# Alandroid/img-compression-mps

Hardware: AMD Instinct MI355X
Metric: Mvoxels/s compress+reconstruct, 256^3 fp32, bond chi=64; SSIM vs ref (higher is better)
Workload: dtype f32

## Files before the change

img-compression-mps_amd/csrc/gemm.hip:

```cpp
#include <stdlib.h>

#include <algorithm>

#include <mutex>
#include <type_traits>

#include "common.h"

namespace {

typedef float f32x16 __attribute__((ext_vector_type(16)));
typedef double f64x4 __attribute__((ext_vector_type(4)));

template <typename T>
struct Mfma;

template <>
struct Mfma<float> {
  static constexpr int MT = 32;
  static constexpr int KS = 2;
  static constexpr int NACC = 16;
  typedef f32x16 acc_t;
  static __device__ __forceinline__ acc_t mma(float a, float b, acc_t c) {
    return __builtin_amdgcn_mfma_f32_32x32x2f32(a, b, c, 0, 0, 0);
  }
  static __device__ __forceinline__ int acc_row(int reg, int lane) {
    return (reg & 3) + 8 * (reg >> 2) + 4 * (lane >> 5);
  }
  static __device__ __forceinline__ int acc_col(int lane) { return lane & 31; }
  static __device__ __forceinline__ int frag_idx(int lane) { return lane & 31; }
  static __device__ __forceinline__ int frag_k(int lane) { return lane >> 5; }
};

template <>
struct Mfma<double> {
  static constexpr int MT = 16;
  static constexpr int KS = 4;
  static constexpr int NACC = 4;
  typedef f64x4 acc_t;
  static __device__ __forceinline__ acc_t mma(double a, double b, acc_t c) {
    return __builtin_amdgcn_mfma_f64_16x16x4f64(a, b, c, 0, 0, 0);
  }
  static __device__ __forceinline__ int acc_row(int reg, int lane) { return (lane >> 4) + 4 * reg; }
  static __device__ __forceinline__ int acc_col(int lane) { return lane & 15; }
  static __device__ __forceinline__ int frag_idx(int lane) { return lane & 15; }
  static __device__ __forceinline__ int frag_k(int lane) { return lane >> 4; }
};

template <typename T>
struct alignas(sizeof(T) * 4) Quad {
  T v[4];
};

struct GemmIndex {
  const int64_t* a_row;
  const int64_t* a_col;
  const int64_t* c_row;
  const int64_t* c_col;
  int guarded;
};
inline int gemm_guarded_env() { return getenv("NDMPS_GEMM_GUARDED") ? 1 : 0; }

constexpr int kGemmMaxBatch = 64;
struct GemmBatchPtrs {
  const void* a[kGemmMaxBatch];
  const void* b[kGemmMaxBatch];
  void* c[kGemmMaxBatch];
};

template <typename T, int BM, int BN, int WAVES_M, int WAVES_N, bool TA, bool TB, bool VEC, bool IDX>
__device__ __forceinline__ void
gemm_body(int64_t M, int64_t N, int64_t K, const T* __restrict__ A, int64_t lda, const T* __restrict__ B, int64_t ldb,
          T* __restrict__ C, int64_t ldc, const GemmIndex& ix) {
  using MF = Mfma<T>;
  constexpr int BK = 16;
  constexpr int MT = MF::MT;
  constexpr int TM = BM / (WAVES_M * MT);
  constexpr int TN = BN / (WAVES_N * MT);
  constexpr int PAD = 4;
  constexpr int A_PER = BM * BK / 256, B_PER = BN * BK / 256;
  static_assert(WAVES_M * WAVES_N == 4, "4 waves per workgroup");
  static_assert(TM >= 1 && TN >= 1, "tile too small");
  constexpr bool VA = VEC && A_PER % 4 == 0, VB = VEC && B_PER % 4 == 0;

  __shared__ T As[BK][BM + PAD];
  __shared__ T Bs[BK][BN + PAD];

  const int tid = threadIdx.x;
  const int lane = tid & 63;
  const int wave = tid >> 6;
  const int wm = wave / WAVES_N;
  const int wn = wave % WAVES_N;
  const int64_t m0 = (int64_t)blockIdx.x * BM;
  const int64_t n0 = (int64_t)blockIdx.y * BN;

  typename MF::acc_t acc[TM][TN];
#pragma unroll
  for (int i = 0; i < TM; ++i)
#pragma unroll
    for (int j = 0; j < TN; ++j)
#pragma unroll
      for (int r = 0; r < MF::NACC; ++r) acc[i][j][r] = (T)0;

  T ra[A_PER], rb[B_PER];

  constexpr int kIdxK = 1024;
  __shared__ int64_t acol_s[(IDX && !TA && VEC) ? kIdxK : 1];
  int64_t arow_q[(A_PER / 4) > 0 ? (A_PER / 4) : 1];
  const bool idx_fast = IDX && !TA && VA && ix.a_row != nullptr && K <= kIdxK;
  if (IDX && !TA && VA) {
    if (idx_fast) {
      for (int64_t kk = tid; kk < K; kk += 256) acol_s[kk] = ix.a_col[kk];
#pragma unroll
      for (int i = 0; i < A_PER / 4; ++i) {
        const int m = (tid + 256 * i) / (BK / 4);
        arow_q[i] = m0 + m < M ? ix.a_row[m0 + m] : 0;
      }
      __syncthreads();
    }
  }

  const bool inner_a = VA && m0 + BM <= M && !ix.guarded, inner_b = VB && n0 + BN <= N && !ix.guarded;
  auto fetch_a = [&](int64_t k0) {
    if (VA && inner_a && k0 + BK <= K) {
#pragma unroll
      for (int i = 0; i < A_PER / 4; ++i) {
        const int e = tid + 256 * i;
        const T* src;
        if (TA) {
          src = A + (k0 + e / (BM / 4)) * lda + m0 + (e % (BM / 4)) * 4;
        } else {
          const int m = e / (BK / 4), k = (e % (BK / 4)) * 4;
          if (IDX && idx_fast) src = A + arow_q[i] + acol_s[k0 + k];
          else if (IDX && ix.a_row) src = A + ix.a_row[m0 + m] + ix.a_col[k0 + k];
          else src = A + (m0 + m) * lda + k0 + k;
        }
        const Quad<T> q = *reinterpret_cast<const Quad<T>*>(src);
#pragma unroll
        for (int j = 0; j < 4; ++j) ra[4 * i + j] = q.v[j];
      }
    } else if (VA) {
#pragma unroll
      for (int i = 0; i < A_PER / 4; ++i) {
        const int e = tid + 256 * i;
        Quad<T> q;
        q.v[0] = q.v[1] = q.v[2] = q.v[3] = (T)0;
        if (TA) {
          const int k = e / (BM / 4), m = (e % (BM / 4)) * 4;
          if (k0 + k < K && m0 + m < M) q = *reinterpret_cast<const Quad<T>*>(A + (k0 + k) * lda + m0 + m);
        } else {
          const int m = e / (BK / 4), k = (e % (BK / 4)) * 4;
          if (k0 + k < K && m0 + m < M) {
            if (IDX && idx_fast) q = *reinterpret_cast<const Quad<T>*>(A + arow_q[i] + acol_s[k0 + k]);
            else if (IDX && ix.a_row) q = *reinterpret_cast<const Quad<T>*>(A + ix.a_row[m0 + m] + ix.a_col[k0 + k]);
            else q = *reinterpret_cast<const Quad<T>*>(A + (m0 + m) * lda + k0 + k);
          }
        }
#pragma unroll
        for (int j = 0; j < 4; ++j) ra[4 * i + j] = q.v[j];
      }
    } else {
#pragma unroll
      for (int i = 0; i < A_PER; ++i) {
        const int e = tid + 256 * i;
        int m, k;
        if (TA) {
          k = e / BM;
          m = e % BM;
        } else {
          m = e / BK;
          k = e % BK;
        }
        const int64_t gk = k0 + k, gm = m0 + m;
        if (IDX && ix.a_row) ra[i] = (gk < K && gm < M) ? A[ix.a_row[gm] + ix.a_col[gk]] : (T)0;
        else ra[i] = (gk < K && gm < M) ? (TA ? A[gk * lda + gm] : A[gm * lda + gk]) : (T)0;
      }
    }
  };
  auto fetch_b = [&](int64_t k0) {
    if (VB && inner_b && k0 + BK <= K) {
#pragma unroll
      for (int i = 0; i < B_PER / 4; ++i) {
        const int e = tid + 256 * i;
        const T* src = TB ? B + (n0 + e / (BK / 4)) * ldb + k0 + (e % (BK / 4)) * 4
                          : B + (k0 + e / (BN / 4)) * ldb + n0 + (e % (BN / 4)) * 4;
        const Quad<T> q = *reinterpret_cast<const Quad<T>*>(src);
#pragma unroll
        for (int j = 0; j < 4; ++j) rb[4 * i + j] = q.v[j];
      }
    } else if (VB) {
#pragma unroll
      for (int i = 0; i < B_PER / 4; ++i) {
        const int e = tid + 256 * i;
        Quad<T> q;
        q.v[0] = q.v[1] = q.v[2] = q.v[3] = (T)0;
        if (TB) {
          const int n = e / (BK / 4), k = (e % (BK / 4)) * 4;
          if (k0 + k < K && n0 + n < N) q = *reinterpret_cast<const Quad<T>*>(B + (n0 + n) * ldb + k0 + k);
        } else {
          const int k = e / (BN / 4), n = (e % (BN / 4)) * 4;
          if (k0 + k < K && n0 + n < N) q = *reinterpret_cast<const Quad<T>*>(B + (k0 + k) * ldb + n0 + n);
        }
#pragma unroll
        for (int j = 0; j < 4; ++j) rb[4 * i + j] = q.v[j];
      }
    } else {
#pragma unroll
      for (int i = 0; i < B_PER; ++i) {
        const int e = tid + 256 * i;
        int n, k;
        if (TB) {
          n = e / BK;
          k = e % BK;
        } else {
          k = e / BN;
          n = e % BN;
        }
        const int64_t gk = k0 + k, gn = n0 + n;
        rb[i] = (gk < K && gn < N) ? (TB ? B[gn * ldb + gk] : B[gk * ldb + gn]) : (T)0;
      }
    }
  };
  auto commit = [&]() {
    if (VA) {
#pragma unroll
      for (int i = 0; i < A_PER / 4; ++i) {
        const int e = tid + 256 * i;
        if (TA) {
          const int k = e / (BM / 4), m = (e % (BM / 4)) * 4;
#pragma unroll
          for (int j = 0; j < 4; ++j) As[k][m + j] = ra[4 * i + j];
        } else {
          const int m = e / (BK / 4), k = (e % (BK / 4)) * 4;
#pragma unroll
          for (int j = 0; j < 4; ++j) As[k + j][m] = ra[4 * i + j];
        }
      }
    } else {
#pragma unroll
      for (int i = 0; i < A_PER; ++i) {
        const int e = tid + 256 * i;
        if (TA) As[e / BM][e % BM] = ra[i];
        else As[e % BK][e / BK] = ra[i];
      }
    }
    if (VB) {
#pragma unroll
      for (int i = 0; i < B_PER / 4; ++i) {
        const int e = tid + 256 * i;
        if (TB) {
          const int n = e / (BK / 4), k = (e % (BK / 4)) * 4;
#pragma unroll
          for (int j = 0; j < 4; ++j) Bs[k + j][n] = rb[4 * i + j];
        } else {
          const int k = e / (BN / 4), n = (e % (BN / 4)) * 4;
#pragma unroll
          for (int j = 0; j < 4; ++j) Bs[k][n + j] = rb[4 * i + j];
        }
      }
    } else {
#pragma unroll
      for (int i = 0; i < B_PER; ++i) {
        const int e = tid + 256 * i;
        if (TB) Bs[e % BK][e / BK] = rb[i];
        else Bs[e / BN][e % BN] = rb[i];
      }
    }
  };

  fetch_a(0);
  fetch_b(0);
  const int fi = MF::frag_idx(lane);
  const int fk = MF::frag_k(lane);
  for (int64_t k0 = 0; k0 < K; k0 += BK) {
    __syncthreads();
    commit();
    __syncthreads();
    if (k0 + BK < K) {
      fetch_a(k0 + BK);
      fetch_b(k0 + BK);
    }
#pragma unroll
    for (int kk = 0; kk < BK; kk += MF::KS) {
      T a[TM], b[TN];
#pragma unroll
      for (int i = 0; i < TM; ++i) a[i] = As[kk + fk][(wm * TM + i) * MT + fi];
#pragma unroll
      for (int j = 0; j < TN; ++j) b[j] = Bs[kk + fk][(wn * TN + j) * MT + fi];
#pragma unroll
      for (int i = 0; i < TM; ++i)
#pragma unroll
        for (int j = 0; j < TN; ++j) acc[i][j] = MF::mma(a[i], b[j], acc[i][j]);
    }
  }

  if constexpr (IDX && MF::MT == 32 && BM == 128 && BN == 128 && sizeof(T) == 4) {
    if (ix.c_row) {
      __shared__ float cstage[4][32][36];
      float (*st)[36] = cstage[wave];
      const int rl0 = lane >> 3, cl = (lane & 7) * 4;
      int64_t roff[TM][4], coff[TN][4];
#pragma unroll
      for (int j = 0; j < TN; ++j) {
        const int64_t col = n0 + (wn * TN + j) * MT + cl;
#pragma unroll
        for (int e = 0; e < 4; ++e) coff[j][e] = col + e < N ? ix.c_col[col + e] : -1;
      }
#pragma unroll
      for (int i = 0; i < TM; ++i)
#pragma unroll
        for (int ps = 0; ps < 4; ++ps) {
          const int64_t row = m0 + (wm * TM + i) * MT + rl0 + 8 * ps;
          roff[i][ps] = row < M ? ix.c_row[row] : -1;
        }
#pragma unroll
      for (int i = 0; i < TM; ++i)
#pragma unroll
        for (int j = 0; j < TN; ++j) {
#pragma unroll
          for (int r = 0; r < MF::NACC; ++r) st[MF::acc_row(r, lane)][MF::acc_col(lane)] = acc[i][j][r];
          __builtin_amdgcn_fence(__ATOMIC_RELEASE, "wavefront");
          __builtin_amdgcn_wave_barrier();
          __builtin_amdgcn_fence(__ATOMIC_ACQUIRE, "wavefront");
          const bool run = coff[j][0] >= 0 && coff[j][3] == coff[j][0] + 3 && coff[j][1] == coff[j][0] + 1 &&
                           coff[j][2] == coff[j][0] + 2;
#pragma unroll
          for (int ps = 0; ps < 4; ++ps) {
            const float4 v = *reinterpret_cast<const float4*>(&st[rl0 + 8 * ps][cl]);
            const int64_t ro = roff[i][ps];
            if (ro < 0) continue;
            if (run && ((ro + coff[j][0]) & 3) == 0) {
              *reinterpret_cast<float4*>(C + ro + coff[j][0]) = v;
            } else {
              if (coff[j][0] >= 0) C[ro + coff[j][0]] = v.x;
              if (coff[j][1] >= 0) C[ro + coff[j][1]] = v.y;
              if (coff[j][2] >= 0) C[ro + coff[j][2]] = v.z;
              if (coff[j][3] >= 0) C[ro + coff[j][3]] = v.w;
            }
          }
          __builtin_amdgcn_fence(__ATOMIC_RELEASE, "wavefront");
          __builtin_amdgcn_wave_barrier();
        }
      return;
    }
  }
  if (IDX && ix.c_row) {
    int64_t roff[TM][MF::NACC], coff[TN];
#pragma unroll
    for (int j = 0; j < TN; ++j) {
      const int64_t col = n0 + (wn * TN + j) * MT + MF::acc_col(lane);
      coff[j] = col < N ? ix.c_col[col] : -1;
    }
#pragma unroll
    for (int i = 0; i < TM; ++i)
#pragma unroll
      for (int r = 0; r < MF::NACC; ++r) {
        const int64_t row = m0 + (wm * TM + i) * MT + MF::acc_row(r, lane);
        roff[i][r] = row < M ? ix.c_row[row] : -1;
      }
#pragma unroll
    for (int i = 0; i < TM; ++i)
#pragma unroll
      for (int j = 0; j < TN; ++j)
#pragma unroll
        for (int r = 0; r < MF::NACC; ++r)
          if (roff[i][r] >= 0 && coff[j] >= 0) C[roff[i][r] + coff[j]] = acc[i][j][r];
    return;
  }
#pragma unroll
  for (int i = 0; i < TM; ++i)
#pragma unroll
    for (int j = 0; j < TN; ++j) {
      const int64_t col = n0 + (wn * TN + j) * MT + MF::acc_col(lane);
#pragma unroll
      for (int r = 0; r < MF::NACC; ++r) {
        const int64_t row = m0 + (wm * TM + i) * MT + MF::acc_row(r, lane);
        if (row < M && col < N) C[row * ldc + col] = acc[i][j][r];
      }
    }
}

template <typename T, int BM, int BN, int WAVES_M, int WAVES_N, bool TA, bool TB, bool VEC, bool IDX = false>
__global__ void __launch_bounds__(256, 2)
gemm_kernel(int64_t M, int64_t N, int64_t K, const T* __restrict__ A, int64_t lda,
            const T* __restrict__ B, int64_t ldb, T* __restrict__ C, int64_t ldc, GemmIndex ix = GemmIndex()) {
  gemm_body<T, BM, BN, WAVES_M, WAVES_N, TA, TB, VEC, IDX>(M, N, K, A, lda, B, ldb, C, ldc, ix);
}

template <typename T, int BM, int BN, int WAVES_M, int WAVES_N, bool TA, bool TB, bool VEC, bool IDX = false>
__global__ void __launch_bounds__(256, 2)
gemm_batched_kernel(int64_t M, int64_t N, int64_t K, GemmBatchPtrs p, int64_t lda, int64_t ldb, int64_t ldc,
                    GemmIndex ix = GemmIndex()) {
  gemm_body<T, BM, BN, WAVES_M, WAVES_N, TA, TB, VEC, IDX>(M, N, K, static_cast<const T*>(p.a[blockIdx.z]), lda,
                                                           static_cast<const T*>(p.b[blockIdx.z]), ldb,
                                                           static_cast<T*>(p.c[blockIdx.z]), ldc, ix);
}

template <typename T, int BM, int BN, int WAVES_M, int WAVES_N>
int launch_gemm(int transA, int transB, int64_t m, int64_t n, int64_t k, const T* A, int64_t lda,
                const T* B, int64_t ldb, T* C, int64_t ldc, hipStream_t stream, const GemmBatchPtrs* bp = nullptr,
                int batch = 1) {
  dim3 grid((unsigned)ndmps::ceil_div(m, BM), (unsigned)ndmps::ceil_div(n, BN), (unsigned)batch);
  dim3 block(256);
  GemmIndex gi{nullptr, nullptr, nullptr, nullptr, gemm_guarded_env()};
  const uintptr_t al = sizeof(T) * 4;
  bool vec = lda % 4 == 0 && ldb % 4 == 0 && k % 4 == 0 && (!transA || m % 4 == 0) && (transB || n % 4 == 0);
  if (bp) {
    for (int z = 0; z < batch; ++z) vec = vec && (uintptr_t)bp->a[z] % al == 0 && (uintptr_t)bp->b[z] % al == 0;
  } else {
    vec = vec && (uintptr_t)A % al == 0 && (uintptr_t)B % al == 0;
  }
#define NDMPS_GEMM_LAUNCH(TA_, TB_, V_)                                                                            \
  do {                                                                                                              \
    if (bp)                                                                                                         \
      hipLaunchKernelGGL((gemm_batched_kernel<T, BM, BN, WAVES_M, WAVES_N, TA_, TB_, V_>), grid, block, 0, stream,  \
                         m, n, k, *bp, lda, ldb, ldc, gi);                                                          \
    else                                                                                                            \
      hipLaunchKernelGGL((gemm_kernel<T, BM, BN, WAVES_M, WAVES_N, TA_, TB_, V_>), grid, block, 0, stream, m, n, k,  \
                         A, lda, B, ldb, C, ldc, gi);                                                               \
  } while (0)
#define NDMPS_GEMM_TRANS(V_)                                     \
  do {                                                           \
    if (transA && transB) NDMPS_GEMM_LAUNCH(true, true, V_);     \
    else if (transA) NDMPS_GEMM_LAUNCH(true, false, V_);         \
    else if (transB) NDMPS_GEMM_LAUNCH(false, true, V_);         \
    else NDMPS_GEMM_LAUNCH(false, false, V_);                    \
  } while (0)
  if (vec) NDMPS_GEMM_TRANS(true);
  else NDMPS_GEMM_TRANS(false);
#undef NDMPS_GEMM_TRANS
#undef NDMPS_GEMM_LAUNCH
  NDMPS_LAUNCH_CHECK();
  return NDMPS_OK;
}

template <typename T>
int gemm_check(int64_t m, int64_t n, int64_t k, const T* A, int64_t lda, int transA, const T* B,
               int64_t ldb, int transB, T* C, int64_t ldc) {
  NDMPS_REQUIRE(m >= 0 && n >= 0 && k >= 0, "negative GEMM extent");
  NDMPS_REQUIRE(A && B && C, "NULL GEMM operand");
  NDMPS_REQUIRE(lda >= (transA ? m : k) && ldb >= (transB ? k : n) && ldc >= n,
                "leading dimension too small (lda=%lld ldb=%lld ldc=%lld)", (long long)lda,
                (long long)ldb, (long long)ldc);
  NDMPS_REQUIRE(ndmps::ceil_div(n, 16) < 65536, "GEMM n=%lld exceeds grid.y", (long long)n);
  NDMPS_REQUIRE(ndmps::ceil_div(m, 32) < 2147483647LL, "GEMM m=%lld exceeds grid.x", (long long)m);
  return NDMPS_OK;
}

template <int T, typename TIN>
__global__ void __launch_bounds__(256, 2)
gram_partial_kernel(const TIN* __restrict__ A, int64_t m, int64_t n, int64_t lda,
                    double* __restrict__ partial, int n_tiles_1d, int64_t rows_per_slab) {
  constexpr int TS = 16 * T;
  __shared__ double red[TS][TS + 1];

  int tile = blockIdx.x, ti = 0;
  while (tile >= n_tiles_1d - ti) {
    tile -= n_tiles_1d - ti;
    ++ti;
  }
  const int tj = ti + tile;
  const int64_t i0 = (int64_t)ti * TS, j0 = (int64_t)tj * TS;
  const int64_t slab = blockIdx.y;
  const int64_t r_begin = slab * rows_per_slab;
  const int64_t r_end = min(m, r_begin + rows_per_slab);

  const int tid = threadIdx.x, lane = tid & 63, wave = tid >> 6;
  const int lr = lane >> 4, lc = lane & 15;

  f64x4 acc[T][T];
#pragma unroll
  for (int a = 0; a < T; ++a)
#pragma unroll
    for (int b = 0; b < T; ++b) acc[a][b] = (f64x4){0.0, 0.0, 0.0, 0.0};

  for (int64_t r = r_begin + 4 * wave; r < r_end; r += 16) {
    const int64_t row = r + lr;
    const bool row_ok = row < r_end;
    double av[T], bv[T];
#pragma unroll
    for (int a = 0; a < T; ++a) {
      const int64_t ca = i0 + 16 * a + lc;
      const int64_t cb = j0 + 16 * a + lc;
      av[a] = (row_ok && ca < n) ? ndmps::to_f64(A[row * lda + ca]) : 0.0;
      bv[a] = (row_ok && cb < n) ? ndmps::to_f64(A[row * lda + cb]) : 0.0;
    }
#pragma unroll
    for (int a = 0; a < T; ++a)
#pragma unroll
      for (int b = 0; b < T; ++b)
        acc[a][b] = __builtin_amdgcn_mfma_f64_16x16x4f64(av[a], bv[b], acc[a][b], 0, 0, 0);
  }

  for (int w = 0; w < 4; ++w) {
    if (wave == w) {
#pragma unroll
      for (int a = 0; a < T; ++a)
#pragma unroll
        for (int b = 0; b < T; ++b)
#pragma unroll
          for (int reg = 0; reg < 4; ++reg) {
            const int rr = 16 * a + lr + 4 * reg, cc = 16 * b + lc;
            if (w == 0) red[rr][cc] = acc[a][b][reg];
            else red[rr][cc] += acc[a][b][reg];
          }
    }
    __syncthreads();
  }
  double* out = partial + ((int64_t)slab * gridDim.x + blockIdx.x) * (TS * TS);
  for (int e = tid; e < TS * TS; e += 256) out[e] = red[e / TS][e % TS];
}

template <int TS>
__global__ void __launch_bounds__(256)
tile_reduce_kernel(const double* __restrict__ partial, int n_slabs, int per_group, int n_tiles_1d,
                   int n_tiles, double* __restrict__ out, double* __restrict__ G, int64_t n, int final,
                   const int32_t* __restrict__ perm = nullptr) {
  const int e = blockIdx.y * 256 + threadIdx.x;
  if (e >= TS * TS) return;
  const int s0 = blockIdx.z * per_group, s1 = min(n_slabs, s0 + per_group);
  const double* src = partial + (int64_t)blockIdx.x * (TS * TS) + e;
  const int64_t slab_stride = (int64_t)n_tiles * (TS * TS);
  double s = 0.0;
  int sl = s0;
  for (; sl + 4 <= s1; sl += 4) {
    const double v0 = src[(sl + 0) * slab_stride], v1 = src[(sl + 1) * slab_stride];
    const double v2 = src[(sl + 2) * slab_stride], v3 = src[(sl + 3) * slab_stride];
    s = (((s + v0) + v1) + v2) + v3;
  }
  for (; sl < s1; ++sl) s += src[sl * slab_stride];
  if (!final) {
    out[((int64_t)blockIdx.z * n_tiles + blockIdx.x) * (TS * TS) + e] = s;
    return;
  }
  int tile = blockIdx.x, ti = 0;
  while (tile >= n_tiles_1d - ti) {
    tile -= n_tiles_1d - ti;
    ++ti;
  }
  const int tj = ti + tile;
  const int64_t r = (int64_t)ti * TS + e / TS, c = (int64_t)tj * TS + e % TS;
  if (r < n && c < n && (ti != tj || c >= r)) {
    const int64_t pr = perm ? perm[r] : r, pc = perm ? perm[c] : c;
    G[pr * n + pc] = s;
    G[pc * n + pr] = s;
  }
// ... 525 lines not shown
    for (int a = 0; a < (ROLE == 2 ? 2 : 4); ++a)
#pragma unroll
      for (int b = 0; b < 4; ++b) {
        if (ROLE == 1 && a > b) continue;
#pragma unroll
        for (int reg = 0; reg < 4; ++reg) {
          const int rr = a_col + 16 * a + lr + 4 * reg, cc = b_col + 16 * b + lc;
          out[rr * 128 + cc] = acc[4 * a + b][reg];
        }
      }
  };
  if (!diag) run(std::integral_constant<int, 0>{});
  else if (wave == 0 || wave == 3) run(std::integral_constant<int, 1>{});
  else run(std::integral_constant<int, 2>{});
}

__global__ void __launch_bounds__(256)
gram128_reduce_kernel(const double* __restrict__ partial, Gram128Geom g, double* __restrict__ G, int64_t stride_G, int64_t n,
                      const int32_t* __restrict__ perm) {
  const int e = blockIdx.y * 256 + threadIdx.x;
  const int t = blockIdx.x;
  int ti, tj, base, count;
  if (t < g.n_off) {
    int u = t;
    ti = 0;
    while (u >= g.tiles_1d - 1 - ti) {
      u -= g.tiles_1d - 1 - ti;
      ++ti;
    }
    tj = ti + 1 + u;
    base = t * g.slabs_off;
    count = g.slabs_off;
  } else {
    ti = tj = t - g.n_off;
    base = g.n_off * g.slabs_off + (t - g.n_off) * g.slabs_diag;
    count = g.slabs_diag;
  }
  const int64_t r = (int64_t)ti * 128 + e / 128, c = (int64_t)tj * 128 + e % 128;
  if (r >= n || c >= n || (ti == tj && c < r)) return;
  const double* src = partial + ((int64_t)blockIdx.z * g.slots + base) * (128 * 128) + e;
  double s = 0.0;
  int sl = 0;
  for (; sl + 4 <= count; sl += 4) {
    const double v0 = src[(int64_t)(sl + 0) * 16384], v1 = src[(int64_t)(sl + 1) * 16384];
    const double v2 = src[(int64_t)(sl + 2) * 16384], v3 = src[(int64_t)(sl + 3) * 16384];
    s = (((s + v0) + v1) + v2) + v3;
  }
  for (; sl < count; ++sl) s += src[(int64_t)sl * 16384];
  double* Gb = G + (int64_t)blockIdx.z * stride_G;
  const int64_t pr = perm ? perm[r] : r, pc = perm ? perm[c] : c;
  Gb[pr * n + pc] = s;
  Gb[pc * n + pr] = s;
}

template <typename TIN>
__global__ void __launch_bounds__(256)
gram_small_kernel(const TIN* __restrict__ A, int64_t m, int n, int64_t lda, double* __restrict__ partial,
                  int vec_ok) {
  __shared__ double red[4][36];
  double acc[36];
#pragma unroll
  for (int i = 0; i < 36; ++i) acc[i] = 0.0;
  const int64_t stride = (int64_t)gridDim.x * 256;
  for (int64_t r = (int64_t)blockIdx.x * 256 + threadIdx.x; r < m; r += stride) {
    float x[8];
    const TIN* row = A + r * lda;
    if (vec_ok) {
      const float4 a = load4_as_f32(row), b = load4_as_f32(row + 4);
      x[0] = a.x; x[1] = a.y; x[2] = a.z; x[3] = a.w; x[4] = b.x; x[5] = b.y; x[6] = b.z; x[7] = b.w;
    } else {
#pragma unroll
      for (int c = 0; c < 8; ++c) x[c] = c < n ? (float)row[c] : 0.f;
    }
    int idx = 0;
#pragma unroll
    for (int i = 0; i < 8; ++i)
#pragma unroll
      for (int j = i; j < 8; ++j) acc[idx++] += (double)x[i] * (double)x[j];
  }
#pragma unroll
  for (int i = 0; i < 36; ++i) {
    double v = acc[i];
    for (int off = 32; off > 0; off >>= 1) v += __shfl_down(v, off, 64);
    if ((threadIdx.x & 63) == 0) red[threadIdx.x >> 6][i] = v;
  }
  __syncthreads();
  if (threadIdx.x < 36)
    partial[(int64_t)blockIdx.x * 36 + threadIdx.x] =
        (red[0][threadIdx.x] + red[1][threadIdx.x]) + (red[2][threadIdx.x] + red[3][threadIdx.x]);
}

__global__ void __launch_bounds__(256)
gram_small_reduce_kernel(const double* __restrict__ partial, int n_blocks, double* __restrict__ G, int n) {
  __shared__ double part[7][36];
  const int e = threadIdx.x % 36, grp = threadIdx.x / 36;
  if (grp < 7) {
    double acc = 0.0;
    for (int b = grp; b < n_blocks; b += 7) acc += partial[(int64_t)b * 36 + e];
    part[grp][e] = acc;
  }
  __syncthreads();
  if (threadIdx.x >= 36) return;
  double s = 0.0;
  for (int k = 0; k < 7; ++k) s += part[k][e];
  int i = 0, rem = e;
  while (rem >= 8 - i) {
    rem -= 8 - i;
    ++i;
  }
  const int j = i + rem;
  if (i < n && j < n) {
    G[i * n + j] = s;
    G[j * n + i] = s;
  }
}

constexpr int kGramSmallBlocks = 256;

struct GramGeom {
  int T;
  int tiles_1d;
  int n_tiles;
  int n_slabs;
  int64_t rows_per_slab;
};

GramGeom gram_geometry(int64_t m, int64_t n) {
  GramGeom g;
  g.T = n <= 16 ? 1 : (n <= 32 ? 2 : 4);
  const int ts = 16 * g.T;
  g.tiles_1d = (int)ndmps::ceil_div(n, ts);
  g.n_tiles = g.tiles_1d * (g.tiles_1d + 1) / 2;
  int64_t want = std::max<int64_t>(1, (2 * ndmps::kNumCU) / g.n_tiles);
  int64_t rows = ndmps::round_up(std::max<int64_t>(ndmps::ceil_div(m, want), 64), 16);
  g.rows_per_slab = rows;
  g.n_slabs = (int)std::max<int64_t>(1, ndmps::ceil_div(m, rows));
  return g;
}

}

extern "C" int ndmps_sgemm(int transA, int transB, int64_t m, int64_t n, int64_t k, const float* d_A,
                           int64_t lda, const float* d_B, int64_t ldb, float* d_C, int64_t ldc,
                           ndmps_stream_t stream) {
  NDMPS_TRY(gemm_check(m, n, k, d_A, lda, transA, d_B, ldb, transB, d_C, ldc));
  if (m == 0 || n == 0) return NDMPS_OK;
  hipStream_t s = (hipStream_t)stream;
  if (n <= 32) return launch_gemm<float, 128, 32, 4, 1>(transA, transB, m, n, k, d_A, lda, d_B, ldb, d_C, ldc, s);
  if (n <= 64 || m <= 64)
    return launch_gemm<float, 64, 64, 2, 2>(transA, transB, m, n, k, d_A, lda, d_B, ldb, d_C, ldc, s);
  return launch_gemm<float, 128, 128, 2, 2>(transA, transB, m, n, k, d_A, lda, d_B, ldb, d_C, ldc, s);
}

extern "C" int ndmps_sgemm_indexed(int64_t m, int64_t n, int64_t k, const float* d_A, int64_t lda,
                                   const int64_t* d_a_row, const int64_t* d_a_col, int a_vec4, const float* d_B,
                                   int64_t ldb, float* d_C, int64_t ldc, const int64_t* d_c_row,
                                   const int64_t* d_c_col, ndmps_stream_t stream) {
  NDMPS_REQUIRE(m >= 0 && n >= 0 && k >= 0 && d_A && d_B && d_C, "bad indexed GEMM argument");
  NDMPS_REQUIRE((d_a_row == nullptr) == (d_a_col == nullptr) && (d_c_row == nullptr) == (d_c_col == nullptr),
                "offset tables come in (row, column) pairs");
  NDMPS_REQUIRE(ldb >= n && (d_a_row || lda >= k) && (d_c_row || ldc >= n), "leading dimension too small");
  if (m == 0 || n == 0) return NDMPS_OK;
  hipStream_t s = (hipStream_t)stream;
  GemmIndex ix{d_a_row, d_a_col, d_c_row, d_c_col, gemm_guarded_env()};
  const uintptr_t al = 16;
  const bool vec = ldb % 4 == 0 && k % 4 == 0 && n % 4 == 0 && (uintptr_t)d_A % al == 0 && (uintptr_t)d_B % al == 0 &&
                   (d_a_row ? a_vec4 != 0 : lda % 4 == 0);
  const dim3 block(256);
  if (n <= 64 || m <= 64) {
    const dim3 grid((unsigned)ndmps::ceil_div(m, 64), (unsigned)ndmps::ceil_div(n, 64));
    if (vec)
      hipLaunchKernelGGL((gemm_kernel<float, 64, 64, 2, 2, false, false, true, true>), grid, block, 0, s, m, n, k, d_A,
                         lda, d_B, ldb, d_C, ldc, ix);
    else
      hipLaunchKernelGGL((gemm_kernel<float, 64, 64, 2, 2, false, false, false, true>), grid, block, 0, s, m, n, k, d_A,
                         lda, d_B, ldb, d_C, ldc, ix);
  } else {
    const dim3 grid((unsigned)ndmps::ceil_div(m, 128), (unsigned)ndmps::ceil_div(n, 128));
    if (vec)
      hipLaunchKernelGGL((gemm_kernel<float, 128, 128, 2, 2, false, false, true, true>), grid, block, 0, s, m, n, k,
                         d_A, lda, d_B, ldb, d_C, ldc, ix);
    else
      hipLaunchKernelGGL((gemm_kernel<float, 128, 128, 2, 2, false, false, false, true>), grid, block, 0, s, m, n, k,
                         d_A, lda, d_B, ldb, d_C, ldc, ix);
  }
  NDMPS_LAUNCH_CHECK();
  return NDMPS_OK;
}

extern "C" int ndmps_dgemm(int transA, int transB, int64_t m, int64_t n, int64_t k, const double* d_A,
                           int64_t lda, const double* d_B, int64_t ldb, double* d_C, int64_t ldc,
                           ndmps_stream_t stream) {
  NDMPS_TRY(gemm_check(m, n, k, d_A, lda, transA, d_B, ldb, transB, d_C, ldc));
  if (m == 0 || n == 0) return NDMPS_OK;
  hipStream_t s = (hipStream_t)stream;
  if (n <= 16) return launch_gemm<double, 64, 16, 4, 1>(transA, transB, m, n, k, d_A, lda, d_B, ldb, d_C, ldc, s);
  if (n <= 32 || m <= 32)
    return launch_gemm<double, 32, 32, 2, 2>(transA, transB, m, n, k, d_A, lda, d_B, ldb, d_C, ldc, s);
  return launch_gemm<double, 64, 64, 2, 2>(transA, transB, m, n, k, d_A, lda, d_B, ldb, d_C, ldc, s);
}

namespace {
template <typename T>
int gemm_batched_check(int batch, const T* const* h_A, const T* const* h_B, T* const* h_C, GemmBatchPtrs& bp) {
  NDMPS_REQUIRE(batch >= 1 && batch <= kGemmMaxBatch && h_A && h_B && h_C, "batched GEMM: batch=%d outside [1, %d] or NULL array",
                batch, kGemmMaxBatch);
  for (int z = 0; z < batch; ++z) {
    NDMPS_REQUIRE(h_A[z] && h_B[z] && h_C[z], "batched GEMM: NULL operand %d", z);
    bp.a[z] = h_A[z];
    bp.b[z] = h_B[z];
    bp.c[z] = h_C[z];
  }
  return NDMPS_OK;
}
}

extern "C" int ndmps_gemm_batched_max(void) { return kGemmMaxBatch; }

extern "C" int ndmps_sgemm_batched(int batch, int transA, int transB, int64_t m, int64_t n, int64_t k,
                                   const float* const* h_A, int64_t lda, const float* const* h_B, int64_t ldb,
                                   float* const* h_C, int64_t ldc, ndmps_stream_t stream) {
  GemmBatchPtrs bp;
  NDMPS_TRY(gemm_batched_check(batch, h_A, h_B, h_C, bp));
  NDMPS_TRY(gemm_check(m, n, k, h_A[0], lda, transA, h_B[0], ldb, transB, h_C[0], ldc));
  if (m == 0 || n == 0) return NDMPS_OK;
  hipStream_t s = (hipStream_t)stream;
  const float* A = nullptr;
  float* Cn = nullptr;
  if (n <= 32) return launch_gemm<float, 128, 32, 4, 1>(transA, transB, m, n, k, A, lda, A, ldb, Cn, ldc, s, &bp, batch);
  if (n <= 64 || m <= 64)
    return launch_gemm<float, 64, 64, 2, 2>(transA, transB, m, n, k, A, lda, A, ldb, Cn, ldc, s, &bp, batch);
  return launch_gemm<float, 128, 128, 2, 2>(transA, transB, m, n, k, A, lda, A, ldb, Cn, ldc, s, &bp, batch);
}

extern "C" int ndmps_dgemm_batched(int batch, int transA, int transB, int64_t m, int64_t n, int64_t k,
                                   const double* const* h_A, int64_t lda, const double* const* h_B, int64_t ldb,
                                   double* const* h_C, int64_t ldc, ndmps_stream_t stream) {
  GemmBatchPtrs bp;
  NDMPS_TRY(gemm_batched_check(batch, h_A, h_B, h_C, bp));
  NDMPS_TRY(gemm_check(m, n, k, h_A[0], lda, transA, h_B[0], ldb, transB, h_C[0], ldc));
  if (m == 0 || n == 0) return NDMPS_OK;
  hipStream_t s = (hipStream_t)stream;
  const double* A = nullptr;
  double* Cn = nullptr;
  if (n <= 16) return launch_gemm<double, 64, 16, 4, 1>(transA, transB, m, n, k, A, lda, A, ldb, Cn, ldc, s, &bp, batch);
  if (n <= 32 || m <= 32)
    return launch_gemm<double, 32, 32, 2, 2>(transA, transB, m, n, k, A, lda, A, ldb, Cn, ldc, s, &bp, batch);
  return launch_gemm<double, 64, 64, 2, 2>(transA, transB, m, n, k, A, lda, A, ldb, Cn, ldc, s, &bp, batch);
}

namespace {
template <int NB>
__global__ void __launch_bounds__(256, 2)
proj64_stream_kernel(GemmBatchPtrs ptrs, int64_t m, int64_t ldb, int64_t ldc, const int64_t* __restrict__ row_sorted,
                     const int32_t* __restrict__ row_order, const int64_t* __restrict__ col_off, int64_t tiles_per_wg) {
  constexpr int N = 32 * NB, Q = 8;
  const float* A = static_cast<const float*>(ptrs.a[blockIdx.z]);
  const float* W = static_cast<const float*>(ptrs.b[blockIdx.z]);
  float* C = static_cast<float*>(ptrs.c[blockIdx.z]);
  __shared__ __attribute__((aligned(16))) float Wp[Q * 2 * N * 4];
  const int tid = threadIdx.x, lane = tid & 63, wave = tid >> 6;
  for (int e = tid; e < 64 * N; e += 256) {
    const int kidx = e / N, j = e % N;
    const int q = kidx >> 3, h = (kidx >> 2) & 1, c = kidx & 3;
    Wp[((q * 2 + h) * N + j) * 4 + c] = W[(int64_t)kidx * ldb + j];
  }
  __syncthreads();
  const int li = lane & 31, h = lane >> 5;
  int64_t coff[Q];
#pragma unroll
  for (int q = 0; q < Q; ++q) coff[q] = col_off[8 * q + 4 * h];
  const int64_t n_tiles = (m + 31) / 32;
  const int64_t t_begin = (int64_t)blockIdx.y * tiles_per_wg, t_end = min(n_tiles, t_begin + tiles_per_wg);
  auto row_offset = [&](int64_t t) { return row_sorted[min(32 * t + li, m - 1)]; };
  int64_t t = t_begin + wave;
  if (t >= t_end) return;
  float4 ring[Q];
  int64_t roff = row_offset(t), roff_next = row_offset(t + 4);
#pragma unroll
  for (int q = 0; q < Q; ++q) ring[q] = load4_stream_f32(A + roff + coff[q]);
  for (; t < t_end; t += 4) {
    f32x16 acc[NB];
#pragma unroll
    for (int nb = 0; nb < NB; ++nb)
#pragma unroll
      for (int r = 0; r < 16; ++r) acc[nb][r] = 0.0f;
    const int64_t roff_after = row_offset(t + 8);
    int crow_of[16];
#pragma unroll
    for (int r = 0; r < 16; ++r) crow_of[r] = row_order[min(32 * t + (r & 3) + 8 * (r >> 2) + 4 * h, m - 1)];
#pragma unroll
    for (int q = 0; q < Q; ++q) {
      float4 a = ring[q];
      asm volatile("" : "+v"(a.x), "+v"(a.y), "+v"(a.z), "+v"(a.w));
      float4 bq[NB];
#pragma unroll
      for (int nb = 0; nb < NB; ++nb) bq[nb] = *reinterpret_cast<const float4*>(&Wp[((q * 2 + h) * N + 32 * nb + li) * 4]);
      __builtin_amdgcn_sched_barrier(0);
      ring[q] = load4_stream_f32(A + roff_next + coff[q]);
#pragma unroll
      for (int nb = 0; nb < NB; ++nb) {
        acc[nb] = __builtin_amdgcn_mfma_f32_32x32x2f32(a.x, bq[nb].x, acc[nb], 0, 0, 0);
        acc[nb] = __builtin_amdgcn_mfma_f32_32x32x2f32(a.y, bq[nb].y, acc[nb], 0, 0, 0);
        acc[nb] = __builtin_amdgcn_mfma_f32_32x32x2f32(a.z, bq[nb].z, acc[nb], 0, 0, 0);
        acc[nb] = __builtin_amdgcn_mfma_f32_32x32x2f32(a.w, bq[nb].w, acc[nb], 0, 0, 0);
      }
      __builtin_amdgcn_sched_barrier(0);
    }
    roff_next = roff_after;
#pragma unroll
    for (int r = 0; r < 16; ++r) {
      const int64_t s = 32 * t + (r & 3) + 8 * (r >> 2) + 4 * h;
      if (s < m) {
        float* crow = C + (int64_t)crow_of[r] * ldc + li;
#pragma unroll
        for (int nb = 0; nb < NB; ++nb) crow[32 * nb] = acc[nb][r];
      }
    }
  }
}

}

extern "C" int ndmps_sgemm_indexed_batched(int batch, int64_t m, int64_t n, int64_t k, const float* const* h_A,
                                           int64_t lda, const int64_t* d_a_row, const int64_t* d_a_col, int a_vec4,
                                           const float* const* h_B, int64_t ldb, float* const* h_C, int64_t ldc,
                                           const int64_t* d_c_row, const int64_t* d_c_col, ndmps_stream_t stream) {
  GemmBatchPtrs bp;
  NDMPS_TRY(gemm_batched_check(batch, h_A, h_B, h_C, bp));
  NDMPS_REQUIRE(m >= 0 && n >= 0 && k >= 0, "bad indexed GEMM extent");
  NDMPS_REQUIRE((d_a_row == nullptr) == (d_a_col == nullptr) && (d_c_row == nullptr) == (d_c_col == nullptr),
                "offset tables come in (row, column) pairs");
  NDMPS_REQUIRE(ldb >= n && (d_a_row || lda >= k) && (d_c_row || ldc >= n), "leading dimension too small");
  if (m == 0 || n == 0) return NDMPS_OK;
  hipStream_t s = (hipStream_t)stream;
  GemmIndex ix{d_a_row, d_a_col, d_c_row, d_c_col, gemm_guarded_env()};
  const uintptr_t al = 16;
  bool vec = ldb % 4 == 0 && k % 4 == 0 && n % 4 == 0 && (d_a_row ? a_vec4 != 0 : lda % 4 == 0);
  for (int z = 0; z < batch; ++z) vec = vec && (uintptr_t)bp.a[z] % al == 0 && (uintptr_t)bp.b[z] % al == 0;
  const dim3 block(256);
  if (n <= 64 || m <= 64) {
    const dim3 grid((unsigned)ndmps::ceil_div(m, 64), (unsigned)ndmps::ceil_div(n, 64), (unsigned)batch);
    if (vec)
      hipLaunchKernelGGL((gemm_batched_kernel<float, 64, 64, 2, 2, false, false, true, true>), grid, block, 0, s, m, n, k,
                         bp, lda, ldb, ldc, ix);
    else
      hipLaunchKernelGGL((gemm_batched_kernel<float, 64, 64, 2, 2, false, false, false, true>), grid, block, 0, s, m, n,
                         k, bp, lda, ldb, ldc, ix);
  } else {
    const dim3 grid((unsigned)ndmps::ceil_div(m, 128), (unsigned)ndmps::ceil_div(n, 128), (unsigned)batch);
    if (vec)
      hipLaunchKernelGGL((gemm_batched_kernel<float, 128, 128, 2, 2, false, false, true, true>), grid, block, 0, s, m, n,
                         k, bp, lda, ldb, ldc, ix);
    else
      hipLaunchKernelGGL((gemm_batched_kernel<float, 128, 128, 2, 2, false, false, false, true>), grid, block, 0, s, m,
                         n, k, bp, lda, ldb, ldc, ix);
  }
  NDMPS_LAUNCH_CHECK();
  return NDMPS_OK;
}

extern "C" int ndmps_sgemm_gathered64_stream_batched(int batch, int64_t m, int64_t n, const float* const* h_A,
                                                     const int64_t* d_row_sorted, const int32_t* d_row_order,
                                                     const int64_t* d_col_off, const float* const* h_B, int64_t ldb,
                                                     float* const* h_C, int64_t ldc, ndmps_stream_t stream) {
  GemmBatchPtrs bp;
  NDMPS_TRY(gemm_batched_check(batch, h_A, h_B, h_C, bp));
  NDMPS_REQUIRE(d_row_sorted && d_row_order && d_col_off, "NULL table");
  NDMPS_REQUIRE(m >= 1 && (n == 32 || n == 64) && ldb >= n && ldc >= n, "the stream takes 32 or 64 result columns");
  for (int z = 0; z < batch; ++z) NDMPS_REQUIRE((uintptr_t)bp.a[z] % 16 == 0, "operand %d is not 16-byte aligned", z);
  hipStream_t s = (hipStream_t)stream;
  const int64_t n_tiles = ndmps::ceil_div(m, 32);
  const int64_t want = std::max<int64_t>(1, ndmps::ceil_div((int64_t)4 * ndmps::kNumCU, batch));
  const int64_t tiles_per_wg = ndmps::round_up(std::max<int64_t>(ndmps::ceil_div(n_tiles, want), 4), 4);
  const dim3 grid(1, (unsigned)ndmps::ceil_div(n_tiles, tiles_per_wg), (unsigned)batch);
  if (n == 32)
    hipLaunchKernelGGL(proj64_stream_kernel<1>, grid, dim3(256), 0, s, bp, m, ldb, ldc, d_row_sorted, d_row_order, d_col_off,
                       tiles_per_wg);
  else
    hipLaunchKernelGGL(proj64_stream_kernel<2>, grid, dim3(256), 0, s, bp, m, ldb, ldc, d_row_sorted, d_row_order, d_col_off,
                       tiles_per_wg);
  NDMPS_LAUNCH_CHECK();
  return NDMPS_OK;
}

inline int gram_wide_tile(int64_t n) { return n >= 128 ? 128 : 64; }

GramGeom gram_wide_geometry(int64_t m, int64_t n) {
  GramGeom g;
  const int GW_TS = gram_wide_tile(n);
  g.T = GW_TS / 16;
  g.tiles_1d = (int)ndmps::ceil_div(n, GW_TS);
  g.n_tiles = g.tiles_1d * (g.tiles_1d + 1) / 2;
  const int64_t want = std::max<int64_t>(1, (2 * ndmps::kNumCU) / g.n_tiles);
  g.rows_per_slab = ndmps::round_up(std::max<int64_t>(ndmps::ceil_div(m, want), 4 * GW_KB), GW_KB);
  g.n_slabs = (int)std::max<int64_t>(1, ndmps::ceil_div(m, g.rows_per_slab));
  return g;
}

inline bool gram_use_wide(int64_t m, int64_t n) { return n >= 64 && m >= 256; }
inline bool gram_use_small(int64_t n) { return n <= 8; }

inline bool gram_use_128(int64_t m, int64_t n) { return n >= 128 && m >= 256; }

Gram128Geom gram128_geometry(int64_t m, int64_t n, int batch) {
  Gram128Geom g;
  g.tiles_1d = (int)ndmps::ceil_div(n, 128);
  g.n_off = g.tiles_1d * (g.tiles_1d - 1) / 2;
  g.n_diag = g.tiles_1d;
  const double weight = g.n_off + 0.625 * g.n_diag;
  const double want = 2.0 * ndmps::kNumCU * (batch > 1 ? 12.0 : 1.0) / std::max(batch, 1) / weight;
  const int64_t floor_rows = batch > 1 ? 512 : 128;
  int64_t s_off = std::max<int64_t>(1, std::min<int64_t>((int64_t)(want + 0.5), std::max<int64_t>(m / floor_rows, 1)));
  g.rows_off = ndmps::round_up(ndmps::ceil_div(m, s_off), GW_KB);
  g.rows_diag = ndmps::round_up((g.rows_off * 8 + 4) / 5, GW_KB);
  g.slabs_off = (int)ndmps::ceil_div(m, g.rows_off);
  g.slabs_diag = (int)ndmps::ceil_div(m, g.rows_diag);
  g.xcd = 0;
  g.members = g.groups_per_matrix = g.groups_total = 0;
  const char* xe = getenv("NDMPS_GRAM_XCD");
  const int xmode = xe ? atoi(xe) : 0;
  if (batch > 1 && g.tiles_1d >= 2 && g.slabs_off >= 4 && xmode == 1) {
    g.rows_diag = 2 * g.rows_off;
    g.slabs_diag = (int)ndmps::ceil_div(m, g.rows_diag);
    g.xcd = 1;
    g.members = 2 * g.n_off + g.n_diag;
    g.groups_per_matrix = g.slabs_diag;
    g.groups_total = batch * g.groups_per_matrix;
  } else if (batch > 1 && g.tiles_1d >= 2 && g.slabs_off >= 4 && xmode == 2) {
    const int64_t s2 = std::max<int64_t>(1, (int64_t)(g.slabs_off * weight / (g.n_off + g.n_diag) + 0.5));
    g.rows_off = g.rows_diag = ndmps::round_up(ndmps::ceil_div(m, s2), GW_KB);
    g.slabs_off = g.slabs_diag = (int)ndmps::ceil_div(m, g.rows_off);
    g.xcd = 2;
    g.members = g.n_off + g.n_diag;
    g.groups_per_matrix = g.slabs_off;
    g.groups_total = batch * g.groups_per_matrix;
  }
  g.slots = g.n_off * g.slabs_off + g.n_diag * g.slabs_diag;
  return g;
}

inline int64_t gram128_workspace(int64_t m, int64_t n, int batch) {
  return (int64_t)batch * gram128_geometry(m, n, batch).slots * 128 * 128 * (int64_t)sizeof(double) + 256;
}

int gram128_opt_in() {
  static std::mutex mu;
  static bool done[64] = {};
  int dev = 0;
  NDMPS_CHECK_HIP(hipGetDevice(&dev));
  std::lock_guard<std::mutex> lock(mu);
  if (dev < 0 || dev >= 64 || done[dev]) return NDMPS_OK;
#define NDMPS_GRAM128_OPT_IN(T, MODE)                                                                          \
  NDMPS_CHECK_HIP(hipFuncSetAttribute(reinterpret_cast<const void*>(&gram128_kernel<T, MODE>),                 \
                                      hipFuncAttributeMaxDynamicSharedMemorySize, (int)kGram128Lds))
  NDMPS_GRAM128_OPT_IN(float, 0);
  NDMPS_GRAM128_OPT_IN(float, 1);
  NDMPS_GRAM128_OPT_IN(float, 2);
  NDMPS_GRAM128_OPT_IN(__bf16, 0);
  NDMPS_GRAM128_OPT_IN(__bf16, 1);
  NDMPS_GRAM128_OPT_IN(__bf16, 2);
#undef NDMPS_GRAM128_OPT_IN
  done[dev] = true;
  return NDMPS_OK;
}

template <typename TIN>
int gram128_batched(int batch, const TIN* const* h_A, int64_t m, int64_t n, int64_t lda, double* d_G, int64_t stride_G,
                    void* d_ws, int64_t ws_bytes, hipStream_t s, const int64_t* d_row_off, const int64_t* d_col_off,
                    const int32_t* d_perm = nullptr) {
  NDMPS_REQUIRE(batch >= 1 && h_A && d_G && gram_use_128(m, n) && lda >= n && stride_G >= n * n,
                "bad batched Gram argument (batch=%d m=%lld n=%lld)", batch, (long long)m, (long long)n);
  const int64_t need = gram128_workspace(m, n, batch);
  if (!d_ws || ws_bytes < need) {
    ndmps::set_error("Gram workspace too small: %lld < %lld", (long long)ws_bytes, (long long)need);
    return NDMPS_EWORKSPACE;
  }
  NDMPS_TRY(gram128_opt_in());
  const Gram128Geom g = gram128_geometry(m, n, batch);
  int vec_ok = (lda % 4 == 0 && n % 4 == 0) ? 1 : 0;
  for (int b = 0; b < batch; ++b) {
    NDMPS_REQUIRE(h_A[b], "NULL Gram operand %d", b);
    if ((uintptr_t)h_A[b] % (4 * sizeof(TIN)) != 0) vec_ok = 0;
  }
  if (d_row_off)
    NDMPS_REQUIRE(d_col_off && vec_ok, "gathered Gram needs n %% 4 == 0 and aligned bases");
  double* partial = (double*)d_ws;
  const bool turn = (int64_t)batch * g.slots >= 4096 && !getenv("NDMPS_GRAM_NO_TURN");
  static const bool one_turn = getenv("NDMPS_ONE_TURN") != nullptr;
  ndmps::Turn gram_turn(s, one_turn ? ndmps::kTurnTeam : ndmps::kTurnGram, one_turn ? 2u : 1u, one_turn ? 2u : 1u);
  if (turn) NDMPS_TRY(gram_turn.begin());
  void* span = ndmps::span_begin(s);
  for (int base = 0; base < batch; base += kGram128MaxBatch) {
    const int count = std::min(kGram128MaxBatch, batch - base);
    Gram128Ptrs ptrs;
    for (int t = 0; t < count; ++t) ptrs.a[t] = h_A[base + t];
    const bool interior = vec_ok && n % 128 == 0 && m % GW_KB == 0 && g.rows_off % GW_KB == 0 && g.rows_diag % GW_KB == 0 &&
                          !getenv("NDMPS_GRAM_GENERAL");
    auto kernel = !interior ? gram128_kernel<TIN, 0> : (d_row_off ? gram128_kernel<TIN, 2> : gram128_kernel<TIN, 1>);
    if (g.xcd) {
      Gram128Geom gc = g;
      gc.groups_total = count * g.groups_per_matrix;
      const unsigned wgs = (unsigned)(ndmps::ceil_div(gc.groups_total, 8) * g.members * 8);
      hipLaunchKernelGGL(kernel, dim3(wgs), dim3(256), kGram128Lds, s, ptrs, m, n, lda,
                         partial + (int64_t)base * g.slots * 16384, gc, vec_ok, d_row_off, d_col_off);
    } else {
      hipLaunchKernelGGL(kernel, dim3(g.slots, count), dim3(256), kGram128Lds, s, ptrs, m, n, lda,
                         partial + (int64_t)base * g.slots * 16384, g, vec_ok, d_row_off, d_col_off);
    }
  }
// ... 231 lines not shown
```

Baseline: 41830.

## Replace indexed GEMM scatter epilogue with block-staged, row-sorted coalesced stores

The old epilogue staged each 32x32 accumulator tile per wave in shared memory and scattered float4s using per-lane offset tables, and it only covered 128x128 tiles. The new SCAT path stages a full BM x 32 column strip for the whole workgroup. It sorts the tile's destination rows by their output offset with a rank count in shared memory. It then picks the widest contiguous column-run granularity with a ballot and issues stores in sorted-row order, so consecutive lanes write to adjacent addresses. It also extends to 64x64 tiles. The cost is extra __syncthreads, more shared memory use that may reduce occupancy, and the per-tile sorting work.

```diff
diff --git a/img-compression-mps_amd/csrc/gemm.hip b/img-compression-mps_amd/csrc/gemm.hip
--- a/img-compression-mps_amd/csrc/gemm.hip
+++ b/img-compression-mps_amd/csrc/gemm.hip
@@ -68,7 +68,7 @@
   void* c[kGemmMaxBatch];
 };
 
-template <typename T, int BM, int BN, int WAVES_M, int WAVES_N, bool TA, bool TB, bool VEC, bool IDX>
+template <typename T, int BM, int BN, int WAVES_M, int WAVES_N, bool TA, bool TB, bool VEC, bool IDX, bool SCAT>
 __device__ __forceinline__ void
 gemm_body(int64_t M, int64_t N, int64_t K, const T* __restrict__ A, int64_t lda, const T* __restrict__ B, int64_t ldb,
           T* __restrict__ C, int64_t ldc, const GemmIndex& ix) {
@@ -294,55 +294,80 @@
     }
   }
 
-  if constexpr (IDX && MF::MT == 32 && BM == 128 && BN == 128 && sizeof(T) == 4) {
-    if (ix.c_row) {
-      __shared__ float cstage[4][32][36];
-      float (*st)[36] = cstage[wave];
-      const int rl0 = lane >> 3, cl = (lane & 7) * 4;
-      int64_t roff[TM][4], coff[TN][4];
+  if constexpr (SCAT) {
+    static_assert(IDX && std::is_same<T, float>::value && MT == 32 && (BM == 64 || BM == 128) && BN % 32 == 0,
+                  "the scatter epilogue is written for the fp32 tiles");
+    constexpr int LBM = BM == 64 ? 6 : 7;
+    constexpr int SW = 32, SLD = SW + 8;
+    __shared__ __attribute__((aligned(16))) float stage[BM][SLD];
+    __shared__ __attribute__((aligned(16))) int64_t coff_s[SW];
+    __shared__ int64_t roff_s[BM];
+    __shared__ int rank_s[BM];
+    __shared__ unsigned short srow_s[BM];
+    if (tid < BM) {
+      roff_s[tid] = m0 + tid < M ? ix.c_row[m0 + tid] : -1;
+      rank_s[tid] = 0;
+    }
+    __syncthreads();
+    {
+      constexpr int PARTS = 256 / BM, SPAN = BM / PARTS;
+      const int row = tid % BM, part = tid / BM;
+      const int64_t mine = roff_s[row] < 0 ? INT64_MAX : roff_s[row];
+      int below = 0;
+      for (int r = part * SPAN; r < (part + 1) * SPAN; ++r) {
+        const int64_t other = roff_s[r] < 0 ? INT64_MAX : roff_s[r];
+        below += (other < mine || (other == mine && r < row)) ? 1 : 0;
+      }
+      atomicAdd(&rank_s[row], below);
+    }
+    __syncthreads();
+    if (tid < BM) srow_s[rank_s[tid]] = (unsigned short)tid;
+    for (int h = 0; h < BN / SW; ++h) {
+      if (h > 0) __syncthreads();
+      if (tid < SW) {
+        const int64_t col = n0 + h * SW + tid;
+        coff_s[tid] = col < N ? ix.c_col[col] : -1;
+      }
 #pragma unroll
       for (int j = 0; j < TN; ++j) {
-        const int64_t col = n0 + (wn * TN + j) * MT + cl;
-#pragma unroll
-        for (int e = 0; e < 4; ++e) coff[j][e] = col + e < N ? ix.c_col[col + e] : -1;
-      }
-#pragma unroll
-      for (int i = 0; i < TM; ++i)
-#pragma unroll
-        for (int ps = 0; ps < 4; ++ps) {
-          const int64_t row = m0 + (wm * TM + i) * MT + rl0 + 8 * ps;
-          roff[i][ps] = row < M ? ix.c_row[row] : -1;
+        if (wn * TN + j != h) continue;
+#pragma unroll
+        for (int i = 0; i < TM; ++i)
+#pragma unroll
+          for (int r = 0; r < MF::NACC; ++r)
+            stage[(wm * TM + i) * MT + MF::acc_row(r, lane)][MF::acc_col(lane)] = acc[i][j][r];
+      }
+      __syncthreads();
+      const int cl = lane < SW ? lane : SW - 1;
+      const int64_t c_here = coff_s[cl], c_next = coff_s[cl < SW - 1 ? cl + 1 : cl];
+      const unsigned long long breaks =
+          __ballot(lane < SW && (lane == SW - 1 || c_here < 0 || c_next != c_here + 1));
+      int lg = 5;
+      for (; lg > 2; --lg) {
+        unsigned long long ends = 0;
+        for (int c = (1 << lg) - 1; c < SW; c += 1 << lg) ends |= 1ull << c;
+        if ((breaks & ~ends) == 0) break;
+      }
+      const int lq = lg - 2;
+      for (int q = tid; q < BM * (SW / 4); q += 256) {
+        const int g = q >> (LBM + lq), s = (q >> lq) & (BM - 1), cq = (g << lq) + (q & ((1 << lq) - 1));
+        const int row = srow_s[s];
+        const int64_t ro = roff_s[row];
+        if (ro < 0) continue;
+        const float4 v = *reinterpret_cast<const float4*>(&stage[row][cq * 4]);
+        const int64_t c0 = coff_s[cq * 4], c1 = coff_s[cq * 4 + 1], c2 = coff_s[cq * 4 + 2], c3 = coff_s[cq * 4 + 3];
+        float* dst = C + ro + c0;
+        if (c0 >= 0 && c1 == c0 + 1 && c2 == c0 + 2 && c3 == c0 + 3 && ((uintptr_t)dst & 15) == 0) {
+          *reinterpret_cast<float4*>(dst) = v;
+        } else {
+          if (c0 >= 0) C[ro + c0] = v.x;
+          if (c1 >= 0) C[ro + c1] = v.y;
+          if (c2 >= 0) C[ro + c2] = v.z;
+          if (c3 >= 0) C[ro + c3] = v.w;
         }
-#pragma unroll
-      for (int i = 0; i < TM; ++i)
-#pragma unroll
-        for (int j = 0; j < TN; ++j) {
-#pragma unroll
-          for (int r = 0; r < MF::NACC; ++r) st[MF::acc_row(r, lane)][MF::acc_col(lane)] = acc[i][j][r];
-          __builtin_amdgcn_fence(__ATOMIC_RELEASE, "wavefront");
-          __builtin_amdgcn_wave_barrier();
-          __builtin_amdgcn_fence(__ATOMIC_ACQUIRE, "wavefront");
-          const bool run = coff[j][0] >= 0 && coff[j][3] == coff[j][0] + 3 && coff[j][1] == coff[j][0] + 1 &&
-                           coff[j][2] == coff[j][0] + 2;
-#pragma unroll
-          for (int ps = 0; ps < 4; ++ps) {
-            const float4 v = *reinterpret_cast<const float4*>(&st[rl0 + 8 * ps][cl]);
-            const int64_t ro = roff[i][ps];
-            if (ro < 0) continue;
-            if (run && ((ro + coff[j][0]) & 3) == 0) {
-              *reinterpret_cast<float4*>(C + ro + coff[j][0]) = v;
-            } else {
-              if (coff[j][0] >= 0) C[ro + coff[j][0]] = v.x;
-              if (coff[j][1] >= 0) C[ro + coff[j][1]] = v.y;
-              if (coff[j][2] >= 0) C[ro + coff[j][2]] = v.z;
-              if (coff[j][3] >= 0) C[ro + coff[j][3]] = v.w;
-            }
-          }
-          __builtin_amdgcn_fence(__ATOMIC_RELEASE, "wavefront");
-          __builtin_amdgcn_wave_barrier();
-        }
-      return;
-    }
+      }
+    }
+    return;
   }
   if (IDX && ix.c_row) {
     int64_t roff[TM][MF::NACC], coff[TN];
@@ -380,18 +405,20 @@
     }
 }
 
-template <typename T, int BM, int BN, int WAVES_M, int WAVES_N, bool TA, bool TB, bool VEC, bool IDX = false>
+template <typename T, int BM, int BN, int WAVES_M, int WAVES_N, bool TA, bool TB, bool VEC, bool IDX = false,
+          bool SCAT = false>
 __global__ void __launch_bounds__(256, 2)
 gemm_kernel(int64_t M, int64_t N, int64_t K, const T* __restrict__ A, int64_t lda,
             const T* __restrict__ B, int64_t ldb, T* __restrict__ C, int64_t ldc, GemmIndex ix = GemmIndex()) {
-  gemm_body<T, BM, BN, WAVES_M, WAVES_N, TA, TB, VEC, IDX>(M, N, K, A, lda, B, ldb, C, ldc, ix);
-}
-
-template <typename T, int BM, int BN, int WAVES_M, int WAVES_N, bool TA, bool TB, bool VEC, bool IDX = false>
+  gemm_body<T, BM, BN, WAVES_M, WAVES_N, TA, TB, VEC, IDX, SCAT>(M, N, K, A, lda, B, ldb, C, ldc, ix);
+}
+
+template <typename T, int BM, int BN, int WAVES_M, int WAVES_N, bool TA, bool TB, bool VEC, bool IDX = false,
+          bool SCAT = false>
 __global__ void __launch_bounds__(256, 2)
 gemm_batched_kernel(int64_t M, int64_t N, int64_t K, GemmBatchPtrs p, int64_t lda, int64_t ldb, int64_t ldc,
                     GemmIndex ix = GemmIndex()) {
-  gemm_body<T, BM, BN, WAVES_M, WAVES_N, TA, TB, VEC, IDX>(M, N, K, static_cast<const T*>(p.a[blockIdx.z]), lda,
+  gemm_body<T, BM, BN, WAVES_M, WAVES_N, TA, TB, VEC, IDX, SCAT>(M, N, K, static_cast<const T*>(p.a[blockIdx.z]), lda,
                                                            static_cast<const T*>(p.b[blockIdx.z]), ldb,
                                                            static_cast<T*>(p.c[blockIdx.z]), ldc, ix);
 }
@@ -1223,6 +1250,21 @@
   return launch_gemm<float, 128, 128, 2, 2>(transA, transB, m, n, k, d_A, lda, d_B, ldb, d_C, ldc, s);
 }
 
+#define NDMPS_IDX_DISPATCH(SMALL_, VEC_, SCAT_)                      \
+  do {                                                               \
+    const int which_ = ((SMALL_) ? 4 : 0) | ((VEC_) ? 2 : 0) | ((SCAT_) ? 1 : 0); \
+    switch (which_) {                                                \
+      case 0: NDMPS_IDX_LAUNCH(128, false, false); break;            \
+      case 1: NDMPS_IDX_LAUNCH(128, false, true); break;             \
+      case 2: NDMPS_IDX_LAUNCH(128, true, false); break;             \
+      case 3: NDMPS_IDX_LAUNCH(128, true, true); break;              \
+      case 4: NDMPS_IDX_LAUNCH(64, false, false); break;             \
+      case 5: NDMPS_IDX_LAUNCH(64, false, true); break;              \
+      case 6: NDMPS_IDX_LAUNCH(64, true, false); break;              \
+      default: NDMPS_IDX_LAUNCH(64, true, true); break;              \
+    }                                                                \
+  } while (0)
+
 extern "C" int ndmps_sgemm_indexed(int64_t m, int64_t n, int64_t k, const float* d_A, int64_t lda,
                                    const int64_t* d_a_row, const int64_t* d_a_col, int a_vec4, const float* d_B,
                                    int64_t ldb, float* d_C, int64_t ldc, const int64_t* d_c_row,
@@ -1238,23 +1280,14 @@
   const bool vec = ldb % 4 == 0 && k % 4 == 0 && n % 4 == 0 && (uintptr_t)d_A % al == 0 && (uintptr_t)d_B % al == 0 &&
                    (d_a_row ? a_vec4 != 0 : lda % 4 == 0);
   const dim3 block(256);
-  if (n <= 64 || m <= 64) {
-    const dim3 grid((unsigned)ndmps::ceil_div(m, 64), (unsigned)ndmps::ceil_div(n, 64));
-    if (vec)
-      hipLaunchKernelGGL((gemm_kernel<float, 64, 64, 2, 2, false, false, true, true>), grid, block, 0, s, m, n, k, d_A,
-                         lda, d_B, ldb, d_C, ldc, ix);
-    else
-      hipLaunchKernelGGL((gemm_kernel<float, 64, 64, 2, 2, false, false, false, true>), grid, block, 0, s, m, n, k, d_A,
-                         lda, d_B, ldb, d_C, ldc, ix);
-  } else {
-    const dim3 grid((unsigned)ndmps::ceil_div(m, 128), (unsigned)ndmps::ceil_div(n, 128));
-    if (vec)
-      hipLaunchKernelGGL((gemm_kernel<float, 128, 128, 2, 2, false, false, true, true>), grid, block, 0, s, m, n, k,
-                         d_A, lda, d_B, ldb, d_C, ldc, ix);
-    else
-      hipLaunchKernelGGL((gemm_kernel<float, 128, 128, 2, 2, false, false, false, true>), grid, block, 0, s, m, n, k,
-                         d_A, lda, d_B, ldb, d_C, ldc, ix);
-  }
+  const bool small = n <= 64 || m <= 64;
+  const int64_t tile = small ? 64 : 128;
+  const dim3 grid((unsigned)ndmps::ceil_div(m, tile), (unsigned)ndmps::ceil_div(n, tile));
+#define NDMPS_IDX_LAUNCH(TILE_, V_, S_)                                                                              \
+  hipLaunchKernelGGL((gemm_kernel<float, TILE_, TILE_, 2, 2, false, false, V_, true, S_>), grid, block, 0, s, m, n, k, \
+                     d_A, lda, d_B, ldb, d_C, ldc, ix)
+  NDMPS_IDX_DISPATCH(small, vec, d_c_row != nullptr);
+#undef NDMPS_IDX_LAUNCH
   NDMPS_LAUNCH_CHECK();
   return NDMPS_OK;
 }
@@ -1410,23 +1443,15 @@
   bool vec = ldb % 4 == 0 && k % 4 == 0 && n % 4 == 0 && (d_a_row ? a_vec4 != 0 : lda % 4 == 0);
   for (int z = 0; z < batch; ++z) vec = vec && (uintptr_t)bp.a[z] % al == 0 && (uintptr_t)bp.b[z] % al == 0;
   const dim3 block(256);
-  if (n <= 64 || m <= 64) {
-    const dim3 grid((unsigned)ndmps::ceil_div(m, 64), (unsigned)ndmps::ceil_div(n, 64), (unsigned)batch);
-    if (vec)
-      hipLaunchKernelGGL((gemm_batched_kernel<float, 64, 64, 2, 2, false, false, true, true>), grid, block, 0, s, m, n, k,
-                         bp, lda, ldb, ldc, ix);
-    else
-      hipLaunchKernelGGL((gemm_batched_kernel<float, 64, 64, 2, 2, false, false, false, true>), grid, block, 0, s, m, n,
-                         k, bp, lda, ldb, ldc, ix);
-  } else {
-    const dim3 grid((unsigned)ndmps::ceil_div(m, 128), (unsigned)ndmps::ceil_div(n, 128), (unsigned)batch);
-    if (vec)
-      hipLaunchKernelGGL((gemm_batched_kernel<float, 128, 128, 2, 2, false, false, true, true>), grid, block, 0, s, m, n,
-                         k, bp, lda, ldb, ldc, ix);
-    else
-      hipLaunchKernelGGL((gemm_batched_kernel<float, 128, 128, 2, 2, false, false, false, true>), grid, block, 0, s, m,
-                         n, k, bp, lda, ldb, ldc, ix);
-  }
+  const bool small = n <= 64 || m <= 64;
+  const int64_t tile = small ? 64 : 128;
+  const dim3 grid((unsigned)ndmps::ceil_div(m, tile), (unsigned)ndmps::ceil_div(n, tile), (unsigned)batch);
+#define NDMPS_IDX_LAUNCH(TILE_, V_, S_)                                                                             \
+  hipLaunchKernelGGL((gemm_batched_kernel<float, TILE_, TILE_, 2, 2, false, false, V_, true, S_>), grid, block, 0, s, \
+                     m, n, k, bp, lda, ldb, ldc, ix)
+  NDMPS_IDX_DISPATCH(small, vec, d_c_row != nullptr);
+#undef NDMPS_IDX_LAUNCH
+#undef NDMPS_IDX_DISPATCH
   NDMPS_LAUNCH_CHECK();
   return NDMPS_OK;
 }
```

Result: no change. 41570 (-0.6%).
